# thesteve0/llm-fine-tune-distributed

Hardware: AMD Instinct MI355X
Metric: samples/sec SmolLM3-3B full SFT bf16 (DDP) (higher is better)
Workload: dtype bf16

## Files before the change

### csrc/bindings.cpp

```cpp
#include <torch/library.h>

#include <string>
#include <vector>

namespace sftamd {
int64_t ipc_ar_create(int64_t cap, int64_t world, int64_t rank);
std::vector<int64_t> ipc_ar_handle(int64_t id);
void ipc_ar_open(int64_t id, std::vector<int64_t> handles);
int64_t ipc_ar_check(int64_t id);
int64_t ipc_ar_poll(int64_t id);
int64_t ipc_ar_uncached(int64_t id);
void ipc_ar_destroy(int64_t id);
std::vector<int64_t> ddp_plan(std::vector<int64_t> sizes, std::vector<int64_t> region, int64_t tied, int64_t align,
                              int64_t pad_unit, int64_t cap, int64_t first_cap, int64_t split_at);
int64_t ddp_tracker_create(std::vector<int64_t> owner_ptr, std::vector<int64_t> owners, int64_t n_buckets);
void ddp_tracker_reset(int64_t id);
std::vector<int64_t> ddp_tracker_mark(int64_t id, int64_t param);
std::vector<int64_t> ddp_tracker_drain(int64_t id);
std::vector<int64_t> ddp_tracker_pending(int64_t id);
void ddp_tracker_destroy(int64_t id);
void dispatch_trace(bool on);
std::string dispatch_trace_read();
int64_t set_cu_budget(int64_t n);
}

TORCH_LIBRARY(sftamd, m) {
  m.def("ipc_ar_create(int cap, int world, int rank) -> int", &sftamd::ipc_ar_create);
  m.def("ipc_ar_handle(int ctx) -> int[]", &sftamd::ipc_ar_handle);
  m.def("ipc_ar_open(int ctx, int[] handles) -> ()", &sftamd::ipc_ar_open);
  m.def("ipc_ar_check(int ctx) -> int", &sftamd::ipc_ar_check);
  m.def("ipc_ar_poll(int ctx) -> int", &sftamd::ipc_ar_poll);
  m.def("ipc_ar_uncached(int ctx) -> int", &sftamd::ipc_ar_uncached);
  m.def("ipc_ar_destroy(int ctx) -> ()", &sftamd::ipc_ar_destroy);
  m.def("ddp_plan(int[] sizes, int[] region, int tied, int align, int pad_unit, int cap, int first_cap, "
        "int split_at) -> int[]", &sftamd::ddp_plan);
  m.def("ddp_tracker_create(int[] owner_ptr, int[] owners, int n_buckets) -> int", &sftamd::ddp_tracker_create);
  m.def("ddp_tracker_reset(int id) -> ()", &sftamd::ddp_tracker_reset);
  m.def("ddp_tracker_mark(int id, int param) -> int[]", &sftamd::ddp_tracker_mark);
  m.def("ddp_tracker_drain(int id) -> int[]", &sftamd::ddp_tracker_drain);
  m.def("ddp_tracker_pending(int id) -> int[]", &sftamd::ddp_tracker_pending);
  m.def("ddp_tracker_destroy(int id) -> ()", &sftamd::ddp_tracker_destroy);
  m.def("ipc_ar_allreduce(Tensor(a!) x, int ctx, int round, int blocks=16) -> ()");
  m.def("dispatch_trace(bool on) -> ()", &sftamd::dispatch_trace);
  m.def("dispatch_trace_read() -> str", &sftamd::dispatch_trace_read);
  m.def("set_cu_budget(int n) -> int", &sftamd::set_cu_budget);
  m.def("rmsnorm_fwd(Tensor x, Tensor? residual, Tensor weight, float eps, int y_ld=0) -> (Tensor, Tensor, Tensor)");
  m.def("rmsnorm_bwd(Tensor dy, Tensor h, Tensor weight, Tensor rstd, Tensor? dres, Tensor(a!)? dw_out=None, bool accumulate=False) -> (Tensor, Tensor)");
  m.def("swiglu_fwd(Tensor gate_up) -> Tensor");
  m.def("cu_hog(Tensor(a!) sink, int blocks, float usec) -> ()");
  m.def("swiglu_bwd(Tensor dy, Tensor gate_up) -> Tensor");
  m.def("rope_(Tensor(a!) qkv, Tensor cos, Tensor sin, int n_q, int n_kv, int head_dim, bool inverse) -> ()");
  m.def("embedding_fwd(Tensor ids, Tensor weight) -> Tensor");
  m.def("dropout_add(Tensor? a, Tensor b, float p, int seed) -> Tensor");
  m.def("lora_widen(Tensor x, int R, float p, int seed) -> (Tensor, Tensor)");
  m.def("lora_fwd(Tensor x, Tensor A, float s, float p, int seed, int ldX=0, bool save_xd=False, bool swiglu=False) -> (Tensor, Tensor)");
  m.def("lora_bwd_dx(Tensor base, Tensor dxa, Tensor A, float p, int seed, Tensor? gu=None) -> Tensor");
  m.def("lora_tsum(Tensor X, int K, Tensor S, float p, int seed) -> Tensor");
  m.def("lora_fwd_inplace(Tensor(a!) X, int K, Tensor A, float s, float p, int seed) -> ()");
  m.def("lora_dxa(Tensor dy, Tensor Bc, float s) -> Tensor");
  m.def("lora_dxa_blocks(Tensor dy, Tensor Bc, int[] o, int[] rows, int[] c, int r, float s) -> Tensor");
  m.def("lora_grad_out(Tensor sum, Tensor(a!)[] outs, int[] r0, int[] c0, bool tr, int[] accumulate) -> ()");
  m.def("lora_grad_out2(Tensor sa, Tensor(a!)[] oa, int[] ra, int[] ca, bool ta, int[] aa, Tensor sb, "
        "Tensor(b!)[] ob, int[] rb, int[] cb, bool tb, int[] ab) -> ()");
  m.def("copy2d_batch(Tensor desc, int max_elems) -> ()");
  m.def("embedding_bwd(Tensor dy, Tensor sorted_ids, Tensor perm, Tensor(a!) grad_weight) -> ()");
  m.def("ce_fwd(Tensor(a!) logits, Tensor labels, Tensor inv_count, bool write_grad) -> Tensor");
  m.def("flash_fwd(Tensor qkv, Tensor cu_seqlens, int max_seqlen, int n_q, int n_kv, int head_dim, float scale, bool causal) -> (Tensor, Tensor)");
  m.def("flash_bwd(Tensor dout, Tensor qkv, Tensor out, Tensor lse, Tensor cu_seqlens, int max_seqlen, int n_q, int n_kv, int head_dim, float scale, bool causal, Tensor? delta=None) -> Tensor");
  m.def("flash_bwd_rope(Tensor dout, Tensor qkv, Tensor out, Tensor lse, Tensor cu_seqlens, int max_seqlen, int n_q, int n_kv, int head_dim, float scale, bool causal, Tensor cos, Tensor sin, Tensor? delta=None) -> Tensor");
  m.def("decode_attention(Tensor q, Tensor kcache, Tensor vcache, Tensor cache_len, int n_q, int n_kv, float scale) -> Tensor");
  m.def("sample_token(Tensor logits, Tensor(a!) presence, Tensor(b!) state, Tensor(c!)? tok_out, Tensor(d!)? pos_out, Tensor(e!)? len_out, Tensor(f!)? log, float temperature, int top_k, float top_p, float repetition_penalty, bool do_sample, int seed) -> ()");
  m.def("wgrad_gemm(Tensor(a!) out, Tensor dy, Tensor x, bool accumulate, int cfg=14, Tensor(b!)? norm=None) -> ()");
  m.def("wgrad_gemm_multi(Tensor(a!)[] outs, Tensor[] dys, Tensor[] xs, int[] accs, Tensor(b!)[] norms, int split_all=0, int split_left=0) -> ()");
  m.def("wgrad_gemm_pair(Tensor(a!) out0, Tensor dy0, Tensor x0, bool acc0, Tensor(b!)? norm0, Tensor(c!) out1, Tensor dy1, Tensor x1, bool acc1, Tensor(d!)? norm1, int split_all=0) -> ()");
  m.def("dgrad_gemm(Tensor dy, Tensor w, Tensor? gate_up=None, int cfg=14) -> Tensor");
  m.def("dgrad_gemm_delta(Tensor dy, Tensor w, Tensor attn_out) -> (Tensor, Tensor)");
  m.def("gemm_tn(Tensor a, Tensor w, int cfg=0) -> Tensor");
  m.def("gemm_tn_swiglu(Tensor x, Tensor w_gate_up, int cfg=5) -> (Tensor, Tensor)");
  m.def("gemm_tn_rope(Tensor x, Tensor w, Tensor cos, Tensor sin, int rope_cols, int cfg=0) -> Tensor");
  m.def("sumsq(Tensor x) -> Tensor");
  m.def("sumsq_chunks(Tensor x, Tensor chunks) -> Tensor");
  m.def("adamw_flat(Tensor(a!) param, Tensor grad, Tensor(b!)? master, Tensor(c!) exp_avg, Tensor(d!) exp_avg_sq, Tensor clip_coef, float lr, float beta1, float beta2, float eps, float weight_decay, float bc1, float bc2, int sr_seed=0, int sr_offset=0) -> ()");
  m.def("pack_sequences(Tensor tokens, Tensor offsets, Tensor order, int max_tokens, int pad_id, int pad_multiple) -> (Tensor, Tensor, Tensor, Tensor, Tensor)");
  m.def("pad_batch(Tensor tokens, Tensor offsets, Tensor order, int pad_id, int pad_multiple, int max_length) -> (Tensor, Tensor, Tensor)");
}
```

### csrc/gemm_dgrad.hip

```cpp
#include "common.h"

#include <type_traits>

namespace sftamd {
namespace dgrad {

constexpr int NT = 512;
constexpr int BK = 32;
constexpr int AROWB = 256;
constexpr int AIMG = BK * AROWB;
constexpr int BROWB = 64;

enum { EPI_PLAIN = 0, EPI_SWIGLU_BWD = 1 };

__device__ __forceinline__ int swz_a(int row, int ch) { return ch ^ (((row & 3) << 2) | ((row >> 2) & 3)); }
__device__ __forceinline__ int img_a(int row, int ch) { return row * AROWB + 16 * swz_a(row, ch); }
__device__ __forceinline__ int swz_b(int row, int ch) { return ch ^ ((0x78 >> (2 * ((row >> 2) & 3))) & 3); }

__device__ __forceinline__ void glds16(const u16* src, char* dst) {
  __builtin_amdgcn_global_load_lds((const void __attribute__((address_space(1)))*)src,
                                   (void __attribute__((address_space(3)))*)dst, 16, 0, 0);
}

typedef __attribute__((address_space(3))) s16x4 lds_s4;

__device__ __forceinline__ bf16x8 lds_tr4(const char* base, int off, int offh) {
  s16x4 lo = __builtin_amdgcn_ds_read_tr16_b64_v4i16((lds_s4*)(base + off));
  s16x4 hi = __builtin_amdgcn_ds_read_tr16_b64_v4i16((lds_s4*)(base + offh));
  typedef __attribute__((ext_vector_type(8))) short s16x8;
  s16x8 v = {lo[0], lo[1], lo[2], lo[3], hi[0], hi[1], hi[2], hi[3]};
  return __builtin_bit_cast(bf16x8, v);
}


constexpr unsigned waitcnt_imm(int vm, int lgkm) {
  return (unsigned)((vm & 15) | (7 << 4) | ((lgkm & 15) << 8) | ((vm >> 4) << 14));
}

template <int BM, int BN, int WM, int WN, int NS_>
struct Cfg {
  static constexpr int NS = NS_;
  static constexpr int NW = WM * WN;
  static constexpr int TM = BM / WM, TN = BN / WN;
  static constexpr int FM = TM / 16, FN = TN / 16;
  static constexpr int IA = BM / 128;
  static constexpr int QA = 8 / NW;
  static constexpr int STAGE_A = IA * AIMG, STAGE = STAGE_A + BN * BROWB;
  static constexpr int PB = BN / (16 * NW);
  static constexpr int PPW = IA * QA + PB;
  static constexpr int EPI_LD = TM + 4;
  static constexpr int EPI = NW * 16 * EPI_LD * 4;
  static constexpr int LDS = (NS * STAGE > EPI) ? NS * STAGE : EPI;
  static_assert((NW == 8 || NW == 4) && BM % 128 == 0 && BN % (16 * NW) == 0 && FM >= PPW, "config");
  static_assert(LDS <= 160 * 1024, "LDS budget");
};

template <class G>
struct Stager {
  const u16* pa;
  const u16* pb;
  long lda, ldb;
  int w, left;
  __device__ __forceinline__ void init(const u16* W, const u16* dY, long ldw, long ldd, int n0, int m0, int wave,
                                       int lane, int nsteps) {
    w = wave;
    lda = ldw;
    ldb = ldd;
    left = nsteps;
    const int ra = 4 * wave + (lane >> 4), ca = lane & 15;
    pa = W + (long)ra * ldw + n0 + 8 * swz_a(ra, ca);
    const int rb = lane >> 2;
    pb = dY + (long)(m0 + 16 * wave + rb) * ldd + 8 * swz_b(rb, lane & 3);
  }
  __device__ __forceinline__ void piece(char* buf, int j) {
    if (j < G::IA * G::QA) {
      const int img = j % G::IA, q = j / G::IA;
      glds16(pa + img * 128 + (long)(4 * G::NW * q) * lda, buf + img * AIMG + (w + G::NW * q) * 1024);
    } else {
      const int jj = j - G::IA * G::QA;
      glds16(pb + (long)(16 * G::NW * jj) * ldb, buf + G::STAGE_A + (w + G::NW * jj) * 1024);
    }
  }
  __device__ __forceinline__ void advance() {
    if (--left > 0) {
      pa += BK * lda;
      pb += BK;
    }
  }
  __device__ __forceinline__ void issue(char* buf) {
#pragma unroll
    for (int j = 0; j < G::PPW; ++j) piece(buf, j);
    advance();
  }
};

__device__ __forceinline__ char* pick(int i, char* b0, char* b1, char* b2, char* b3, char* b4) {
  switch (i) {
    case 0: return b0;
    case 1: return b1;
    case 2: return b2;
    case 3: return b3;
    default: return b4;
  }
}

template <class G, bool SCHED>
__device__ __forceinline__ void ring_loop(char* __restrict__ b0, char* __restrict__ b1, char* __restrict__ b2,
                                          char* __restrict__ b3, char* __restrict__ b4, int nsteps, Stager<G>& st,
                                          const int (&offA)[G::FM], const int (&offH)[G::FM], int offB,
                                          f32x4 (&acc)[G::FM][G::FN]) {
  constexpr int NS = G::NS, PPW = G::PPW;
  constexpr int U = (NS % 2) ? 2 * NS : NS;
  bf16x8 fa[G::FM], fb[2][G::FN];
#pragma unroll
  for (int i = 0; i < NS; ++i) st.issue(pick(i, b0, b1, b2, b3, b4));
  __builtin_amdgcn_s_waitcnt(waitcnt_imm((NS - 1) * PPW, 0));
  __builtin_amdgcn_s_barrier();
#pragma unroll
  for (int j = 0; j < G::FN; ++j) fb[0][j] = *(const bf16x8*)(b0 + offB + 1024 * j);
#pragma unroll
  for (int i = 0; i < G::FM; ++i) fa[i] = lds_tr4(b0, offA[i], offH[i]);
  for (int t0 = 0; t0 < nsteps; t0 += U) {
#pragma unroll
    for (int u = 0; u < U; ++u) {
      if (t0 + u < nsteps) {
        __builtin_amdgcn_s_waitcnt(waitcnt_imm((NS - 2) * PPW, 0));
        __builtin_amdgcn_s_barrier();
        char* dst = pick(u % NS, b0, b1, b2, b3, b4);
        const char* nxt = pick((u + 1) % NS, b0, b1, b2, b3, b4);
        const int cb = u & 1;
#pragma unroll
        for (int j = 0; j < G::FN; ++j) fb[cb ^ 1][j] = *(const bf16x8*)(nxt + offB + 1024 * j);
        __builtin_amdgcn_s_setprio(1);
#pragma unroll
        for (int i = 0; i < G::FM; ++i) {
#pragma unroll
          for (int j = 0; j < G::FN; ++j)
            acc[i][j] = __builtin_amdgcn_mfma_f32_16x16x32_bf16(fa[i], fb[cb][j], acc[i][j], 0, 0, 0);
          fa[i] = lds_tr4(nxt, offA[i], offH[i]);
          if (i < PPW) st.piece(dst, i);
          if (SCHED) {
            __builtin_amdgcn_sched_group_barrier(0x008, G::FN, 0);
            __builtin_amdgcn_sched_group_barrier(0x100, 2, 0);
            if (i < PPW) __builtin_amdgcn_sched_group_barrier(0x020, 1, 0);
          }
        }
        st.advance();
        __builtin_amdgcn_s_setprio(0);
      }
    }
  }
  __builtin_amdgcn_s_waitcnt(waitcnt_imm(0, 0));
}

struct EpiArgs {
  u16* out;
  const u16* gu;
  long ldo;
  int N;
};

template <class G, int EPI>
__device__ __forceinline__ void epilogue(char* smem, f32x4 (&acc)[G::FM][G::FN], const EpiArgs& ea, int n0, int m0,
                                         int wm, int wn, int w, int lane) {
  const int g = lane >> 4, c = lane & 15;
  float* ep = reinterpret_cast<float*>(smem) + w * 16 * G::EPI_LD;
  constexpr int SEGS = G::TM / 8;
  if constexpr (EPI == EPI_SWIGLU_BWD) {
    constexpr int IT = 16 * SEGS / 64, U = G::FN * IT, PD = U < 4 ? U : 4;
    static_assert(U >= PD, "ring deeper than the epilogue");
    auto base_of = [&](int u) -> long {
      const int jf = u / IT, seg = (u - jf * IT) * 64 + lane, row = seg / SEGS, cs = seg - row * SEGS;
      const long m = m0 + wn * G::TN + 16 * jf + row;
      return m * 2L * ea.N + n0 + wm * G::TM + cs * 8;
    };
    uint4 rg[PD][2];
#pragma unroll
    for (int u = 0; u < PD; ++u) {
      const long b = base_of(u);
      rg[u][0] = *(const uint4*)(ea.gu + b);
      rg[u][1] = *(const uint4*)(ea.gu + b + ea.N);
    }
#pragma unroll
    for (int jf = 0; jf < G::FN; ++jf) {
#pragma unroll
      for (int i = 0; i < G::FM; ++i) *(f32x4*)(ep + c * G::EPI_LD + 16 * i + 4 * g) = acc[i][jf];
      asm volatile("s_waitcnt lgkmcnt(0)" ::: "memory");
#pragma unroll
      for (int it = 0; it < IT; ++it) {
        const int u = jf * IT + it;
        const int seg = it * 64 + lane, row = seg / SEGS, cs = seg - row * SEGS;
        const float* pr = ep + row * G::EPI_LD + cs * 8;
        float v[8], gt[8], up[8], dg[8], du[8];
        *(float4*)&v[0] = *(const float4*)pr;
        *(float4*)&v[4] = *(const float4*)(pr + 4);
        unpack8(rg[u % PD][0], gt);
        unpack8(rg[u % PD][1], up);
        if (u + PD < U) {
          const long b = base_of(u + PD);
          rg[u % PD][0] = *(const uint4*)(ea.gu + b);
          rg[u % PD][1] = *(const uint4*)(ea.gu + b + ea.N);
        }
#pragma unroll
        for (int e = 0; e < 8; ++e) {
#pragma clang fp contract(off)
          const float sg = 1.f / (1.f + __expf(-gt[e]));
          const float t = v[e] * sg;
          du[e] = t * gt[e];
          dg[e] = (t * up[e]) * __builtin_fmaf(gt[e], 1.f - sg, 1.f);
        }
        const long b = base_of(u);
        *(uint4*)(ea.out + b) = pack8(dg);
        *(uint4*)(ea.out + b + ea.N) = pack8(du);
      }
      asm volatile("s_waitcnt lgkmcnt(0)" ::: "memory");
    }
    return;
  }
#pragma unroll
  for (int jf = 0; jf < G::FN; ++jf) {
#pragma unroll
    for (int i = 0; i < G::FM; ++i) *(f32x4*)(ep + c * G::EPI_LD + 16 * i + 4 * g) = acc[i][jf];
    asm volatile("s_waitcnt lgkmcnt(0)" ::: "memory");
#pragma unroll
    for (int it = 0; it < 16 * SEGS / 64; ++it) {
      const int seg = it * 64 + lane, row = seg / SEGS, cs = seg - row * SEGS;
      const float* pr = ep + row * G::EPI_LD + cs * 8;
      float v[8];
      *(float4*)&v[0] = *(const float4*)pr;
      *(float4*)&v[4] = *(const float4*)(pr + 4);
      const long m = m0 + wn * G::TN + 16 * jf + row;
      const int n = n0 + wm * G::TM + cs * 8;
      if constexpr (EPI == EPI_PLAIN) {
        *(uint4*)(ea.out + m * ea.ldo + n) = pack8(v);
      } else {
        const long base = m * 2L * ea.N + n;
        float gt[8], up[8], dg[8], du[8];
        unpack8(*(const uint4*)(ea.gu + base), gt);
        unpack8(*(const uint4*)(ea.gu + base + ea.N), up);
#pragma unroll
        for (int e = 0; e < 8; ++e) {
          swiglu_grad(v[e], gt[e], up[e], dg[e], du[e]);
        }
        *(uint4*)(ea.out + base) = pack8(dg);
        *(uint4*)(ea.out + base + ea.N) = pack8(du);
      }
    }
    asm volatile("s_waitcnt lgkmcnt(0)" ::: "memory");
  }
}

template <int BM, int BN, int WM, int WN, int NS, int EPI, int OCC = 1, bool SCHED = true>
__global__ void __launch_bounds__(WM * WN * 64, OCC) dgrad_kernel(const u16* __restrict__ dY, const u16* __restrict__ W, int K,
                                                        long ldd, long ldw, int nbn, int nbm, int group, EpiArgs ea) {
  using G = Cfg<BM, BN, WM, WN, NS>;
  __shared__ __attribute__((aligned(16))) char smem[G::LDS];
  const int nwg = gridDim.x, orig = blockIdx.x;
  const int xcd = orig & 7, q8 = nwg >> 3, r8 = nwg & 7;
  const int wgid = (xcd < r8 ? xcd * (q8 + 1) : r8 * (q8 + 1) + (xcd - r8) * q8) + (orig >> 3);
  const int per_group = group * nbm;
  const int grp = wgid / per_group, first = grp * group;
  const int gsz = min(nbn - first, group);
  const int in = wgid - grp * per_group;
  const int bn = first + in % gsz, bm = in / gsz;
  const int n0 = bn * BM, m0 = bm * BN;
  SFT_DASSERT(bn < nbn && bm < nbm);

  const int tid = threadIdx.x, lane = tid & 63, w = __builtin_amdgcn_readfirstlane(tid >> 6);
  const int wm = w / WN, wn = w - wm * WN;

  Stager<G> st;
  st.init(W, dY, ldw, ldd, n0, m0, w, lane, K / BK);
  const int g = lane >> 4, ii = lane & 15, qq = ii >> 2, pp = ii & 3;
  const int r0 = 8 * g + qq;
  int offA[G::FM], offH[G::FM];
#pragma unroll
  for (int i = 0; i < G::FM; ++i) {
    const int nl = wm * G::TM + 16 * i;
    offA[i] = (nl >> 7) * AIMG + img_a(r0, 2 * ((nl & 127) >> 4) + (pp >> 1)) + 8 * (pp & 1);
    offH[i] = (nl >> 7) * AIMG + img_a(r0 + 4, 2 * ((nl & 127) >> 4) + (pp >> 1)) + 8 * (pp & 1);
  }
  const int rowb = wn * G::TN + ii;
  const int offB = G::STAGE_A + rowb * BROWB + 16 * swz_b(ii, g);
  f32x4 acc[G::FM][G::FN];
#pragma unroll
  for (int i = 0; i < G::FM; ++i)
#pragma unroll
    for (int j = 0; j < G::FN; ++j) acc[i][j] = f32x4{0.f, 0.f, 0.f, 0.f};

  char* b[5];
#pragma unroll
  for (int i = 0; i < 5; ++i) b[i] = smem + (i < NS ? i : 0) * G::STAGE;
  ring_loop<G, SCHED>(b[0], b[1], b[2], b[3], b[4], K / BK, st, offA, offH, offB, acc);
  __syncthreads();
  epilogue<G, EPI>(smem, acc, ea, n0, m0, wm, wn, w, lane);
}

constexpr int BK2 = 64;
constexpr int AIMG2 = BK2 * AROWB;
constexpr int BROWB2 = 128;
__device__ __forceinline__ int swz_b2(int row, int ch) { return ch ^ ((row >> 1) & 7); }

template <int BM, int BN, int WM, int WN>
struct Cfg2 {
  static constexpr int NS = 2;
  static constexpr int TM = BM / WM, TN = BN / WN;
  static constexpr int FM = TM / 16, FN = TN / 16;
  static constexpr int IA = BM / 128;
  static constexpr int STAGE_A = IA * AIMG2, STAGE = STAGE_A + BN * BROWB2;
  static constexpr int PA = IA * 2;
  static constexpr int PB = BN / 64;
  static constexpr int PPW = PA + PB;
  static constexpr int EPI_LD = TM + 4;
  static constexpr int EPI = 8 * 16 * EPI_LD * 4;
  static constexpr int LDS = (NS * STAGE > EPI) ? NS * STAGE : EPI;
  static_assert(WM * WN == 8 && BM % 128 == 0 && BN % 64 == 0 && 2 * FM >= PPW, "config");
  static_assert(LDS <= 160 * 1024, "LDS budget");
};

template <class G>
struct Stager2 {
  const u16* pa;
  const u16* pb;
  long lda, ldb;
  int w, left;
  __device__ __forceinline__ void init(const u16* W, const u16* dY, long ldw, long ldd, int n0, int m0, int wave,
                                       int lane, int nsteps) {
    w = wave;
    lda = ldw;
    ldb = ldd;
    left = nsteps;
    const int ra = 4 * wave + (lane >> 4);
    pa = W + (long)ra * ldw + n0 + 8 * swz_a(ra, lane & 15);
    const int rb = 8 * wave + (lane >> 3);
    pb = dY + (long)(m0 + rb) * ldd + 8 * swz_b2(rb, lane & 7);
  }
  __device__ __forceinline__ void piece(char* buf, int j) {
    if (j < G::PA) {
      glds16(pa + (long)(32 * (j & 1)) * lda + 128 * (j >> 1), buf + (j >> 1) * AIMG2 + (w + 8 * (j & 1)) * 1024);
    } else {
      const int jb = j - G::PA;
      glds16(pb + (long)(64 * jb) * ldb, buf + G::STAGE_A + (w + 8 * jb) * 1024);
    }
  }
  __device__ __forceinline__ void advance() {
    if (--left > 0) {
      pa += BK2 * lda;
      pb += BK2;
    }
  }
};

template <class G>
__device__ __forceinline__ void ring2_loop(char* __restrict__ b0, char* __restrict__ b1, int nsteps, Stager2<G>& st,
                                           const int (&offA)[G::FM], const int (&offH)[G::FM], int ob0, int ob1,
                                           f32x4 (&acc)[G::FM][G::FN]) {
  constexpr int PPW = G::PPW;
  bf16x8 fa[G::FM], fb[2][G::FN];
#pragma unroll
  for (int i = 0; i < 2; ++i) {
#pragma unroll
    for (int j = 0; j < PPW; ++j) st.piece(i == 0 ? b0 : b1, j);
    st.advance();
  }
  __builtin_amdgcn_s_waitcnt(waitcnt_imm(PPW, 0));
  __builtin_amdgcn_s_barrier();
#pragma unroll
  for (int j = 0; j < G::FN; ++j) fb[0][j] = *(const bf16x8*)(b0 + ob0 + 2048 * j);
#pragma unroll
  for (int i = 0; i < G::FM; ++i) fa[i] = lds_tr4(b0, offA[i], offH[i]);
  for (int t0 = 0; t0 < nsteps; t0 += 2) {
#pragma unroll
    for (int u = 0; u < 2; ++u) {
      if (t0 + u < nsteps) {
        char* cur = u == 0 ? b0 : b1;
        char* nxt = u == 0 ? b1 : b0;
#pragma unroll
        for (int j = 0; j < G::FN; ++j) fb[1][j] = *(const bf16x8*)(cur + ob1 + 2048 * j);
        __builtin_amdgcn_s_setprio(1);
#pragma unroll
        for (int i = 0; i < G::FM; ++i) {
#pragma unroll
          for (int j = 0; j < G::FN; ++j)
            acc[i][j] = __builtin_amdgcn_mfma_f32_16x16x32_bf16(fa[i], fb[0][j], acc[i][j], 0, 0, 0);
          fa[i] = lds_tr4(cur, offA[i] + 32 * AROWB, offH[i] + 32 * AROWB);
        }
        __builtin_amdgcn_s_setprio(0);
        __builtin_amdgcn_s_waitcnt(waitcnt_imm(0, 0));
        __builtin_amdgcn_s_barrier();
#pragma unroll
        for (int j = 0; j < G::FN; ++j) fb[0][j] = *(const bf16x8*)(nxt + ob0 + 2048 * j);
        __builtin_amdgcn_s_setprio(1);
#pragma unroll
        for (int i = 0; i < G::FM; ++i) {
#pragma unroll
          for (int j = 0; j < G::FN; ++j)
            acc[i][j] = __builtin_amdgcn_mfma_f32_16x16x32_bf16(fa[i], fb[1][j], acc[i][j], 0, 0, 0);
          fa[i] = lds_tr4(nxt, offA[i], offH[i]);
          if (2 * i < PPW) st.piece(cur, 2 * i);
          if (2 * i + 1 < PPW) st.piece(cur, 2 * i + 1);
        }
        st.advance();
        __builtin_amdgcn_s_setprio(0);
      }
    }
  }
  __builtin_amdgcn_s_waitcnt(waitcnt_imm(0, 0));
}

template <int BM, int BN, int WM, int WN, int EPI>
__global__ void __launch_bounds__(NT) dgrad2_kernel(const u16* __restrict__ dY, const u16* __restrict__ W, int K,
                                                    long ldd, long ldw, int nbn, int nbm, int group, EpiArgs ea) {
  using G = Cfg2<BM, BN, WM, WN>;
  __shared__ __attribute__((aligned(16))) char smem[G::LDS];
  const int nwg = gridDim.x, orig = blockIdx.x;
  const int xcd = orig & 7, q8 = nwg >> 3, r8 = nwg & 7;
  const int wgid = (xcd < r8 ? xcd * (q8 + 1) : r8 * (q8 + 1) + (xcd - r8) * q8) + (orig >> 3);
  const int per_group = group * nbm;
  const int grp = wgid / per_group, first = grp * group;
  const int gsz = min(nbn - first, group);
  const int in = wgid - grp * per_group;
  const int bn = first + in % gsz, bm = in / gsz;
  const int n0 = bn * BM, m0 = bm * BN;

  const int tid = threadIdx.x, lane = tid & 63, w = __builtin_amdgcn_readfirstlane(tid >> 6);
  const int wm = w / WN, wn = w - wm * WN;
  Stager2<G> st;
  st.init(W, dY, ldw, ldd, n0, m0, w, lane, K / BK2);
  const int g = lane >> 4, ii = lane & 15, qq = ii >> 2, pp = ii & 3;
  const int r0 = 8 * g + qq;
  int offA[G::FM], offH[G::FM];
#pragma unroll
  for (int i = 0; i < G::FM; ++i) {
    const int nl = wm * G::TM + 16 * i;
    offA[i] = (nl >> 7) * AIMG2 + img_a(r0, 2 * ((nl & 127) >> 4) + (pp >> 1)) + 8 * (pp & 1);
    offH[i] = (nl >> 7) * AIMG2 + img_a(r0 + 4, 2 * ((nl & 127) >> 4) + (pp >> 1)) + 8 * (pp & 1);
  }
  const int rowb = wn * G::TN + ii;
  const int bbase = G::STAGE_A + rowb * BROWB2;
  const int ob0 = bbase + 16 * swz_b2(ii, g), ob1 = bbase + 16 * swz_b2(ii, 4 + g);
  f32x4 acc[G::FM][G::FN];
#pragma unroll
  for (int i = 0; i < G::FM; ++i)
#pragma unroll
    for (int j = 0; j < G::FN; ++j) acc[i][j] = f32x4{0.f, 0.f, 0.f, 0.f};
  ring2_loop<G>(smem, smem + G::STAGE, K / BK2, st, offA, offH, ob0, ob1, acc);
  __syncthreads();
  epilogue<Cfg<BM, BN, WM, WN, 2>, EPI>(smem, acc, ea, n0, m0, wm, wn, w, lane);
}

template <int BM, int BN, int WM, int WN, int EPI>
void launch2(const at::Tensor& dy, const at::Tensor& w, const EpiArgs& ea);

static int group_n() { return 8; }

template <int BM, int BN, int WM, int WN, int NS, int EPI, int OCC = 1, bool SCHED = true>
void launch(const at::Tensor& dy, const at::Tensor& w, const EpiArgs& ea) {
  const int M = dy.size(0), K = dy.size(1), N = w.size(1);
  const int nbn = N / BM, nbm = M / BN;
  dgrad_kernel<BM, BN, WM, WN, NS, EPI, OCC, SCHED><<<nbn * nbm, WM * WN * 64, 0, cur_stream()>>>(
      (const u16*)dy.data_ptr(), (const u16*)w.data_ptr(), K, dy.stride(0), w.stride(0), nbn, nbm,
      std::min(group_n(), nbn), ea);
  SFT_LAUNCH_CHECK();
}

template <int BM, int BN, int WM, int WN, int EPI>
void launch2(const at::Tensor& dy, const at::Tensor& w, const EpiArgs& ea) {
  const int M = dy.size(0), K = dy.size(1), N = w.size(1);
  const int nbn = N / BM, nbm = M / BN;
  dgrad2_kernel<BM, BN, WM, WN, EPI><<<nbn * nbm, NT, 0, cur_stream()>>>(
      (const u16*)dy.data_ptr(), (const u16*)w.data_ptr(), K, dy.stride(0), w.stride(0), nbn, nbm,
      std::min(group_n(), nbn), ea);
  SFT_LAUNCH_CHECK();
}

}

void g4_dgrad(const at::Tensor& dy, const at::Tensor& w, u16* out, long ldo, const u16* attn_out = nullptr,
              long ld_attn = 0, float* delta = nullptr);

std::tuple<at::Tensor, at::Tensor> dgrad_gemm_delta(const at::Tensor& dy, const at::Tensor& w,
                                                    const at::Tensor& attn_out) {
  SFT_CHECK_CUDA(dy);
  SFT_CHECK_BF16(dy);
  SFT_CHECK_BF16(w);
  SFT_CHECK_BF16(attn_out);
  SFT_CHECK(dy.dim() == 2 && w.dim() == 2 && attn_out.dim() == 2, "dgrad_gemm_delta: 2-D operands");
  SFT_CHECK(dy.stride(1) == 1 && w.stride(1) == 1 && attn_out.stride(1) == 1, "dgrad_gemm_delta: contiguous rows");
  const int64_t M = dy.size(0), K = dy.size(1), N = w.size(1);
  SFT_CHECK(w.size(0) == K && attn_out.size(0) == M && attn_out.size(1) == N,
            "dgrad_gemm_delta: dy [M, K] . w [K, N], attn_out [M, N]");
  SFT_CHECK(M % 256 == 0 && N % 256 == 0 && K % 128 == 0 && K > 0 && K < 8192,
            "dgrad_gemm_delta: M, N % 256, K % 128, K < 8192 (whole tiles)");
  SFT_CHECK(dy.stride(0) % 8 == 0 && w.stride(0) % 8 == 0 && (uintptr_t)dy.data_ptr() % 16 == 0 &&
                (uintptr_t)w.data_ptr() % 16 == 0,
            "dgrad_gemm_delta: 16-byte aligned rows");
  auto out = at::empty({M, N}, dy.options());
  auto delta = at::empty({N / 128, M}, dy.options().dtype(at::kFloat));
  SFT_TRACE("dgrad.c14.delta");
  g4_dgrad(dy, w, (u16*)out.data_ptr(), N, (const u16*)attn_out.data_ptr(), attn_out.stride(0),
           delta.data_ptr<float>());
  return {out, delta};
}

at::Tensor dgrad_gemm(const at::Tensor& dy, const at::Tensor& w, const c10::optional<at::Tensor>& gate_up,
                      int64_t cfg) {
  SFT_CHECK_CUDA(dy);
  SFT_CHECK_BF16(dy);
  SFT_CHECK_BF16(w);
  SFT_CHECK(dy.dim() == 2 && w.dim() == 2, "dgrad_gemm: 2-D operands");
  SFT_CHECK(dy.stride(1) == 1 && w.stride(1) == 1, "dgrad_gemm: rows must be contiguous");
  const int64_t M = dy.size(0), K = dy.size(1), N = w.size(1);
  SFT_CHECK(w.size(0) == K, "dgrad_gemm: dy [M, K] . w [K, N]");
  SFT_CHECK(cfg != 7 || K % 64 == 0, "dgrad_gemm cfg 7 (BK 64): K multiple of 64");
  SFT_CHECK(cfg != 14 || K % 128 == 0, "dgrad_gemm cfg 14 (4-wave): K multiple of 128");
  SFT_CHECK(M % 128 == 0 && N % 256 == 0 && K % 32 == 0 && K >= 32, "dgrad_gemm: M multiple of 128 (256 for cfg 0/1), N of 256, K of 32");
  SFT_CHECK(cfg == 2 || M % 256 == 0, "dgrad_gemm: 256 x 256 tiles need M % 256 == 0");
  SFT_CHECK(dy.stride(0) % 8 == 0 && w.stride(0) % 8 == 0 && (uintptr_t)dy.data_ptr() % 16 == 0 &&
                (uintptr_t)w.data_ptr() % 16 == 0,
            "dgrad_gemm: 16-byte aligned rows");
  dgrad::EpiArgs ea{};
  ea.N = (int)N;
  at::Tensor out;
  const bool swiglu = gate_up.has_value() && gate_up->defined();
  if (swiglu) {
    const at::Tensor& gu = *gate_up;
    SFT_CHECK_BF16(gu);
    SFT_CHECK_CONTIG(gu);
    SFT_CHECK(gu.dim() == 2 && gu.size(0) == M && gu.size(1) == 2 * N, "dgrad_gemm: gate_up must be [M, 2N]");
    out = at::empty({M, 2 * N}, dy.options());
    ea.gu = (const u16*)gu.data_ptr();
    ea.ldo = 2 * N;
  } else {
    out = at::empty({M, N}, dy.options());
    ea.ldo = N;
  }
  ea.out = (u16*)out.data_ptr();
  if (M == 0 || N == 0) return out;
  auto run1 = [&](auto epi, int c, const at::Tensor& wv, const dgrad::EpiArgs& e) {
    constexpr int E = decltype(epi)::value;
    SFT_TRACE(trace_name(E == dgrad::EPI_SWIGLU_BWD ? "dgrad.swiglu.c" : "dgrad.c", c));
    switch (c) {
      case 2: dgrad::launch<256, 128, 4, 2, 3, E>(dy, wv, e); break;
      case 5: dgrad::launch<256, 256, 2, 4, 3, E, 1, false>(dy, wv, e); break;
      case 7: dgrad::launch2<256, 256, 2, 4, E>(dy, wv, e); break;
      case 14:
        SFT_CHECK(E == dgrad::EPI_PLAIN, "dgrad_gemm cfg 14: plain epilogue only");
        g4_dgrad(dy, wv, e.out, e.ldo);
        break;
      default: SFT_CHECK(false, "dgrad_gemm: cfg ", c, " not built (2, 5, 7, 14)");
    }
  };
  const int tail_cfg = [] {
    const char* e = std::getenv("SFTAMD_DGRAD_TAIL");
    return e && e[0] ? atoi(e) : 2;
  }();
  auto run = [&](auto epi) {
    const long nbn = N / 256, nbm = M / 256, tiles = nbn * nbm;
    const bool full = cfg != 2;
    long main_n = 0;
    if (full && tail_cfg == 2 && tiles % 256 != 0 && 256 % nbm == 0) {
      main_n = tiles / 256 * (256 / nbm);
      if ((nbn - main_n) * (M / 128) > 256) main_n = 0;
    }
    if (main_n <= 0) {
      run1(epi, (int)cfg, w, ea);
      return;
    }
    const long n_split = main_n * 256;
    SFT_TRACE("dgrad.tail");
    run1(epi, (int)cfg, w.narrow(1, 0, n_split), ea);
    dgrad::EpiArgs et = ea;
    et.out = ea.out + n_split;
    if (et.gu != nullptr) et.gu = ea.gu + n_split;
    run1(epi, tail_cfg, w.narrow(1, n_split, N - n_split), et);
  };
  if (swiglu) run(std::integral_constant<int, dgrad::EPI_SWIGLU_BWD>());
  else run(std::integral_constant<int, dgrad::EPI_PLAIN>());
  return out;
}

TORCH_LIBRARY_IMPL(sftamd, CUDA, m) {
  m.impl("dgrad_gemm", &dgrad_gemm);
  m.impl("dgrad_gemm_delta", &dgrad_gemm_delta);
}

}
```

Measured before the change: 117.7.

## Add persistent dgrad SwiGLU-backward kernel overlapping epilogue drain with next tile's mainloop

Adds a persistent-grid dgrad GEMM for the fused SwiGLU-backward epilogue. Each workgroup parks its accumulators in a global scratch buffer, then drains the previous tile (loading gate/up, computing the SwiGLU gradient, storing) interleaved into the next tile's MFMA ring loop. The goal is to hide the epilogue's memory traffic behind compute when there are more tiles than workgroups. The cost is extra scratch traffic through global memory, a per-call scratch allocation, and intricate hand-placed waitcnt scheduling. The path is taken for cfg 5 with the SwiGLU epilogue whenever the tile count exceeds the CU budget.

```diff
diff --git a/csrc/bindings.cpp b/csrc/bindings.cpp
--- a/csrc/bindings.cpp
+++ b/csrc/bindings.cpp
@@ -73,7 +73,7 @@
   m.def("wgrad_gemm(Tensor(a!) out, Tensor dy, Tensor x, bool accumulate, int cfg=14, Tensor(b!)? norm=None) -> ()");
   m.def("wgrad_gemm_multi(Tensor(a!)[] outs, Tensor[] dys, Tensor[] xs, int[] accs, Tensor(b!)[] norms, int split_all=0, int split_left=0) -> ()");
   m.def("wgrad_gemm_pair(Tensor(a!) out0, Tensor dy0, Tensor x0, bool acc0, Tensor(b!)? norm0, Tensor(c!) out1, Tensor dy1, Tensor x1, bool acc1, Tensor(d!)? norm1, int split_all=0) -> ()");
-  m.def("dgrad_gemm(Tensor dy, Tensor w, Tensor? gate_up=None, int cfg=14) -> Tensor");
+  m.def("dgrad_gemm(Tensor dy, Tensor w, Tensor? gate_up=None, int cfg=14, int wgs=0) -> Tensor");
   m.def("dgrad_gemm_delta(Tensor dy, Tensor w, Tensor attn_out) -> (Tensor, Tensor)");
   m.def("gemm_tn(Tensor a, Tensor w, int cfg=0) -> Tensor");
   m.def("gemm_tn_swiglu(Tensor x, Tensor w_gate_up, int cfg=5) -> (Tensor, Tensor)");
diff --git a/csrc/gemm_dgrad.hip b/csrc/gemm_dgrad.hip
--- a/csrc/gemm_dgrad.hip
+++ b/csrc/gemm_dgrad.hip
@@ -296,6 +296,261 @@
   epilogue<G, EPI>(smem, acc, ea, n0, m0, wm, wn, w, lane);
 }
 
+constexpr int PU = 32;
+constexpr int PARK_VECS = 32 * NT;
+
+struct DrainRegs {
+  f32x4 v;
+  uint2 g, u;
+};
+
+__device__ __forceinline__ unsigned fresh(unsigned x) {
+  asm volatile("" : "+v"(x));
+  return x;
+}
+
+struct Drainer {
+  const char* park;
+  const char* gu;
+  char* out;
+  long ld, tile;
+  unsigned lane_park, lane_gu;
+  int N;
+  __device__ __forceinline__ void init(const char* wave_park, const EpiArgs& ea, int lane) {
+    park = wave_park;
+    gu = (const char*)ea.gu;
+    out = (char*)ea.out;
+    N = ea.N;
+    ld = 2L * ea.N;
+    tile = 0;
+    lane_park = (unsigned)(((lane & 15) >> 2) * 1024 + (16 * (lane & 3) + (lane >> 4)) * 16);
+    lane_gu = (unsigned)(2 * ((lane >> 4) * ld + 4 * (lane & 15)));
+  }
+  __device__ __forceinline__ void set_tile(int n0, int m0, int wm, int wn) {
+    tile = (long)(m0 + wn * 64) * ld + n0 + wm * 128;
+  }
+  __device__ __forceinline__ long offset(int unit) const {
+    const int j = unit >> 3, ih = (unit >> 2) & 1, q4 = unit & 3;
+    return 2 * (tile + (long)(16 * j + 4 * q4) * ld + 64 * ih);
+  }
+  __device__ __forceinline__ void load(int unit, DrainRegs& r) const {
+    const int j = unit >> 3, ih = (unit >> 2) & 1, q4 = unit & 3;
+    r.v = *(const f32x4*)(park + ((j * 8 + 4 * ih) * 1024 + 64 * q4) + fresh(lane_park));
+    const char* p = gu + offset(unit);
+    const unsigned lg = fresh(lane_gu);
+    r.g = *(const uint2*)(p + lg);
+    r.u = *(const uint2*)(p + 2 * N + lg);
+  }
+  __device__ __forceinline__ void load_async(int unit, DrainRegs& r) const {
+    const int j = unit >> 3, ih = (unit >> 2) & 1, q4 = unit & 3;
+    const char* pv = park + ((j * 8 + 4 * ih) * 1024 + 64 * q4);
+    const char* pg = gu + offset(unit);
+    const char* pu = pg + 2 * N;
+    asm volatile("global_load_dwordx4 %0, %1, %2" : "=v"(r.v) : "v"(lane_park), "s"(pv) : "memory");
+    asm volatile("global_load_dwordx2 %0, %1, %2" : "=v"(r.g) : "v"(lane_gu), "s"(pg) : "memory");
+    asm volatile("global_load_dwordx2 %0, %1, %2" : "=v"(r.u) : "v"(lane_gu), "s"(pu) : "memory");
+  }
+  template <int BEHIND>
+  __device__ __forceinline__ void arrived(DrainRegs& r) const {
+    static_assert(BEHIND == 8, "the literal below");
+    asm volatile("s_waitcnt vmcnt(8)" : "+v"(r.v), "+v"(r.g), "+v"(r.u) : : "memory");
+  }
+  __device__ __forceinline__ void math(const DrainRegs& r, int e, float& dg, float& du) const {
+#pragma clang fp contract(off)
+    const unsigned wg = e < 2 ? r.g.x : r.g.y, wu = e < 2 ? r.u.x : r.u.y;
+    const float gt = __uint_as_float((e & 1) ? (wg & 0xffff0000u) : (wg << 16));
+    const float up = __uint_as_float((e & 1) ? (wu & 0xffff0000u) : (wu << 16));
+    const float sg = 1.f / (1.f + __expf(-gt));
+    const float t = r.v[e] * sg;
+    du = t * gt;
+    dg = (t * up) * __builtin_fmaf(gt, 1.f - sg, 1.f);
+  }
+  __device__ __forceinline__ void store(int unit, const float (&dg)[4], const float (&du)[4]) const {
+    char* p = out + offset(unit);
+    const unsigned lg = fresh(lane_gu);
+    *(uint2*)(p + lg) = make_uint2(pk2bf(dg[0], dg[1]), pk2bf(dg[2], dg[3]));
+    *(uint2*)(p + 2 * N + lg) = make_uint2(pk2bf(du[0], du[1]), pk2bf(du[2], du[3]));
+  }
+  __device__ __forceinline__ void finish(int unit, const DrainRegs& r) const {
+    float dg[4], du[4];
+#pragma unroll
+    for (int e = 0; e < 4; ++e) math(r, e, dg[e], du[e]);
+    store(unit, dg, du);
+  }
+  __device__ __forceinline__ void flush(int from) const {
+#pragma unroll 1
+    for (int u0 = from; u0 < PU; u0 += 4) {
+      DrainRegs r[4];
+#pragma unroll
+      for (int k = 0; k < 4; ++k)
+        if (u0 + k < PU) load(u0 + k, r[k]);
+#pragma unroll
+      for (int k = 0; k < 4; ++k)
+        if (u0 + k < PU) finish(u0 + k, r[k]);
+    }
+  }
+};
+
+template <int VM>
+__device__ __forceinline__ void wait_vm() {
+  __builtin_amdgcn_s_waitcnt(waitcnt_imm(VM, 0));
+}
+
+template <class G>
+__device__ __forceinline__ void ring_block(char* __restrict__ b0, char* __restrict__ b1, char* __restrict__ b2, int t0,
+                                           int nsteps, Stager<G>& st, const int (&offA)[G::FM], int dH, int offB,
+                                           f32x4 (&acc)[G::FM][G::FN], bf16x8 (&fa)[G::FM], bf16x8 (&fb)[2][G::FN],
+                                           const Drainer& dr, int unit0) {
+  constexpr int NS = G::NS, PPW = G::PPW;
+  static_assert(NS == 3 && G::FM == 8 && PPW == 4, "ring_block: the 3-stage 256 x 256 ring");
+  DrainRegs r;
+  float dg[4], du[4];
+#pragma unroll
+  for (int u = 0; u < 6; ++u) {
+    if (t0 + u < nsteps) {
+      const bool ld = u % 2 == 0, fin = u % 2 == 1;
+      const int unit = min(unit0 + u / 2, PU - 1);
+      if (ld) wait_vm<PPW + 2>();
+      else wait_vm<PPW + 5>();
+      __builtin_amdgcn_s_barrier();
+      char* dst = pick(u % NS, b0, b1, b2, b0, b0);
+      const char* nxt = pick((u + 1) % NS, b0, b1, b2, b0, b0);
+      const int cb = u & 1;
+#pragma unroll
+      for (int j = 0; j < G::FN; ++j) fb[cb ^ 1][j] = *(const bf16x8*)(nxt + offB + 1024 * j);
+      __builtin_amdgcn_s_setprio(1);
+#pragma unroll
+      for (int i = 0; i < G::FM; ++i) {
+#pragma unroll
+        for (int j = 0; j < G::FN; ++j)
+          acc[i][j] = __builtin_amdgcn_mfma_f32_16x16x32_bf16(fa[i], fb[cb][j], acc[i][j], 0, 0, 0);
+        fa[i] = lds_tr4(nxt, offA[i], offA[i] + (int)fresh((unsigned)dH));
+        if (ld && i == 0) {
+          __builtin_amdgcn_sched_barrier(0);
+          dr.load_async(unit, r);
+          __builtin_amdgcn_sched_barrier(0);
+        }
+        if (i < PPW) st.piece(dst, i);
+        if (fin && i == 4) {
+          __builtin_amdgcn_sched_barrier(0);
+          dr.template arrived<2 * PPW>(r);
+        }
+        if (fin && i >= 4) dr.math(r, i - 4, dg[i - 4], du[i - 4]);
+        if (fin && i == G::FM - 1) {
+          __builtin_amdgcn_sched_barrier(0);
+          dr.store(unit, dg, du);
+          __builtin_amdgcn_sched_barrier(0);
+        }
+      }
+      st.advance();
+      __builtin_amdgcn_s_setprio(0);
+    }
+  }
+}
+
+template <class G>
+__device__ __forceinline__ void ring_fill(char* __restrict__ b0, char* __restrict__ b1, char* __restrict__ b2,
+                                          Stager<G>& st, const int (&offA)[G::FM], int dH, int offB,
+                                          bf16x8 (&fa)[G::FM], bf16x8 (&fb)[2][G::FN], f32x4 (&acc)[G::FM][G::FN],
+                                          char* wave_park, int lane) {
+  st.issue(b0);
+  st.issue(b1);
+  st.issue(b2);
+  __builtin_amdgcn_sched_barrier(0);
+#pragma unroll
+  for (int i = G::FM - 2; i < G::FM; ++i) {
+    *(f32x4*)(wave_park + ((G::FN - 1) * 8 + i) * 1024 + fresh(16 * lane)) = acc[i][G::FN - 1];
+    acc[i][G::FN - 1] = f32x4{0.f, 0.f, 0.f, 0.f};
+  }
+  __builtin_amdgcn_sched_barrier(0);
+  wait_vm<(G::NS - 1) * G::PPW>();
+  __builtin_amdgcn_s_barrier();
+#pragma unroll
+  for (int j = 0; j < G::FN; ++j) fb[0][j] = *(const bf16x8*)(b0 + offB + 1024 * j);
+#pragma unroll
+  for (int i = 0; i < G::FM; ++i) fa[i] = lds_tr4(b0, offA[i], offA[i] + (int)fresh((unsigned)dH));
+}
+
+template <int BM, int BN, int WM, int WN, int NS>
+__device__ __forceinline__ void persistent_body(char* __restrict__ b0, char* __restrict__ b1, char* __restrict__ b2,
+                                                const u16* __restrict__ dY, const u16* __restrict__ W, int K, long ldd,
+                                                long ldw, int nbn, int nbm, int group, const EpiArgs& ea,
+                                                f32x4* scratch) {
+  using G = Cfg<BM, BN, WM, WN, NS>;
+  static_assert(G::NW == 8 && G::TM == 128 && G::TN == 64, "the drain units assume 128 n x 64 m wave tiles");
+  const int tiles = nbn * nbm, q8 = tiles >> 3, r8 = tiles & 7, per_group = group * nbm;
+  const int tid = threadIdx.x, lane = tid & 63, w = __builtin_amdgcn_readfirstlane(tid >> 6);
+  const int wm = w / WN, wn = w - wm * WN;
+  const int g = lane >> 4, ii = lane & 15, qq = ii >> 2, pp = ii & 3;
+  const int r0 = 8 * g + qq;
+  int offA[G::FM];
+#pragma unroll
+  for (int i = 0; i < G::FM; ++i) {
+    const int nl = wm * G::TM + 16 * i;
+    offA[i] = (nl >> 7) * AIMG + img_a(r0, 2 * ((nl & 127) >> 4) + (pp >> 1)) + 8 * (pp & 1);
+  }
+  const int dH = 4 * AROWB + (pp >> 1 ? -16 : 16);
+  const int offB = G::STAGE_A + (wn * G::TN + ii) * BROWB + 16 * swz_b(ii, g);
+  f32x4 acc[G::FM][G::FN];
+#pragma unroll
+  for (int i = 0; i < G::FM; ++i)
+#pragma unroll
+    for (int j = 0; j < G::FN; ++j) acc[i][j] = f32x4{0.f, 0.f, 0.f, 0.f};
+
+  char* wave_park = (char*)(scratch + (long)blockIdx.x * PARK_VECS) + w * 32768;
+  Drainer dr;
+  dr.init(wave_park, ea, lane);
+  const int nsteps = K / BK;
+  bool pending = false;
+  for (int v = blockIdx.x; v < tiles; v += gridDim.x) {
+    const int xcd = v & 7;
+    const int wgid = (xcd < r8 ? xcd * (q8 + 1) : r8 * (q8 + 1) + (xcd - r8) * q8) + (v >> 3);
+    const int grp = wgid / per_group, first = grp * group;
+    const int gsz = min(nbn - first, group);
+    const int in = wgid - grp * per_group;
+    const int bn = first + in % gsz, bm = in / gsz;
+    const int n0 = bn * BM, m0 = bm * BN;
+    SFT_DASSERT(bn < nbn && bm < nbm);
+    Stager<G> st;
+    st.init(W, dY, ldw, ldd, n0, m0, w, lane, nsteps);
+    bf16x8 fa[G::FM], fb[2][G::FN];
+    if (!pending) dr.set_tile(n0, m0, wm, wn);
+    ring_fill<G>(b0, b1, b2, st, offA, dH, offB, fa, fb, acc, wave_park, lane);
+    for (int t0 = 0; t0 < nsteps; t0 += 6)
+      ring_block<G>(b0, b1, b2, t0, nsteps, st, offA, dH, offB, acc, fa, fb, dr, t0 / 2);
+    wait_vm<0>();
+    if (pending) dr.flush(min(nsteps / 2, PU));
+    __syncthreads();
+#pragma unroll
+    for (int j = 0; j < G::FN; ++j)
+#pragma unroll
+      for (int i = 0; i < G::FM; ++i)
+        if (j * 8 + i < 30) {
+          *(f32x4*)(wave_park + (j * 8 + i) * 1024 + fresh(16 * lane)) = acc[i][j];
+          acc[i][j] = f32x4{0.f, 0.f, 0.f, 0.f};
+        }
+    dr.set_tile(n0, m0, wm, wn);
+    pending = true;
+  }
+  if (pending) {
+#pragma unroll
+    for (int i = G::FM - 2; i < G::FM; ++i)
+      *(f32x4*)(wave_park + ((G::FN - 1) * 8 + i) * 1024 + fresh(16 * lane)) = acc[i][G::FN - 1];
+    wait_vm<0>();
+    dr.flush(0);
+  }
+}
+
+template <int BM, int BN, int WM, int WN, int NS>
+__global__ void __launch_bounds__(WM * WN * 64, 1)
+    dgrad_swiglu_persistent_kernel(const u16* __restrict__ dY, const u16* __restrict__ W, int K, long ldd, long ldw,
+                                   int nbn, int nbm, int group, EpiArgs ea, f32x4* scratch) {
+  constexpr int STAGE = Cfg<BM, BN, WM, WN, NS>::STAGE;
+  __shared__ __attribute__((aligned(16))) char smem[NS * STAGE];
+  persistent_body<BM, BN, WM, WN, NS>(smem, smem + STAGE, smem + 2 * STAGE, dY, W, K, ldd, ldw, nbn, nbm, group, ea,
+                                      scratch);
+}
+
 constexpr int BK2 = 64;
 constexpr int AIMG2 = BK2 * AROWB;
 constexpr int BROWB2 = 128;
@@ -461,6 +716,16 @@
   dgrad_kernel<BM, BN, WM, WN, NS, EPI, OCC, SCHED><<<nbn * nbm, WM * WN * 64, 0, cur_stream()>>>(
       (const u16*)dy.data_ptr(), (const u16*)w.data_ptr(), K, dy.stride(0), w.stride(0), nbn, nbm,
       std::min(group_n(), nbn), ea);
+  SFT_LAUNCH_CHECK();
+}
+
+inline void launch_persistent(const at::Tensor& dy, const at::Tensor& w, const EpiArgs& ea, int wgs) {
+  const int M = dy.size(0), K = dy.size(1), N = w.size(1);
+  const int nbn = N / 256, nbm = M / 256;
+  auto scratch = at::empty({(int64_t)wgs * PARK_VECS * 4}, dy.options().dtype(at::kFloat));
+  dgrad_swiglu_persistent_kernel<256, 256, 2, 4, 3><<<wgs, NT, 0, cur_stream()>>>(
+      (const u16*)dy.data_ptr(), (const u16*)w.data_ptr(), K, dy.stride(0), w.stride(0), nbn, nbm,
+      std::min(group_n(), nbn), ea, (f32x4*)scratch.data_ptr());
   SFT_LAUNCH_CHECK();
 }
 
@@ -504,7 +769,7 @@
 }
 
 at::Tensor dgrad_gemm(const at::Tensor& dy, const at::Tensor& w, const c10::optional<at::Tensor>& gate_up,
-                      int64_t cfg) {
+                      int64_t cfg, int64_t wgs) {
   SFT_CHECK_CUDA(dy);
   SFT_CHECK_BF16(dy);
   SFT_CHECK_BF16(w);
@@ -516,6 +781,8 @@
   SFT_CHECK(cfg != 14 || K % 128 == 0, "dgrad_gemm cfg 14 (4-wave): K multiple of 128");
   SFT_CHECK(M % 128 == 0 && N % 256 == 0 && K % 32 == 0 && K >= 32, "dgrad_gemm: M multiple of 128 (256 for cfg 0/1), N of 256, K of 32");
   SFT_CHECK(cfg == 2 || M % 256 == 0, "dgrad_gemm: 256 x 256 tiles need M % 256 == 0");
+  SFT_CHECK(wgs >= 0 && wgs <= 4096, "dgrad_gemm: wgs in [0, 4096]");
+  const int64_t grid = wgs > 0 ? wgs : cu_budget();
   SFT_CHECK(dy.stride(0) % 8 == 0 && w.stride(0) % 8 == 0 && (uintptr_t)dy.data_ptr() % 16 == 0 &&
                 (uintptr_t)w.data_ptr() % 16 == 0,
             "dgrad_gemm: 16-byte aligned rows");
@@ -542,7 +809,10 @@
     SFT_TRACE(trace_name(E == dgrad::EPI_SWIGLU_BWD ? "dgrad.swiglu.c" : "dgrad.c", c));
     switch (c) {
       case 2: dgrad::launch<256, 128, 4, 2, 3, E>(dy, wv, e); break;
-      case 5: dgrad::launch<256, 256, 2, 4, 3, E, 1, false>(dy, wv, e); break;
+      case 5:
+        if (E == dgrad::EPI_SWIGLU_BWD && (M / 256) * (wv.size(1) / 256) > grid) dgrad::launch_persistent(dy, wv, e, (int)grid);
+        else dgrad::launch<256, 256, 2, 4, 3, E, 1, false>(dy, wv, e);
+        break;
       case 7: dgrad::launch2<256, 256, 2, 4, E>(dy, wv, e); break;
       case 14:
         SFT_CHECK(E == dgrad::EPI_PLAIN, "dgrad_gemm cfg 14: plain epilogue only");
```

Measured after the change: 113.6. 0.966x the previous value.
